# numz/ComfyUI-SeedVR2_VideoUpscaler

Measured on AMD Instinct MI355X. Metric: upscaled frames/sec (720p->4K, SeedVR2-3B), higher is better.
Workload: dtype bf16; 1 GPU; cfg3: SeedVR2-3B 32-frame 720p->4K clip (padded to 33 = 4n+1 for encode + DiT, 32 decoded), VAE tiled 1024/128; vae_tiled=True, parallelism=dp1, weights=random-init SeedVR2-3B + video_vae_v3 architecture (seeded)

## Files before the change

### comfyui-seedvr2_videoupscaler_amd/csrc/svr_api.hip

```cpp
#include "svr_common.h"
#include "../../include/seedvr2_hip.h"
#include <cstdio>
#include <vector>
#include <algorithm>
#include <cstring>

#include "svr_gemm.hip"
#include "svr_conv_halo2.hip"
#include "svr_conv_sub.hip"
#include "svr_conv_thinout.hip"
#include "svr_attn_win.hip"
#include "svr_attn.hip"
#include "svr_elementwise.hip"
#include "svr_calibrate.hip"

using namespace svr;

static thread_local char g_err[512] = "";

static int fail(const char* msg) {
    snprintf(g_err, sizeof(g_err), "%s", msg);
    return -1;
}
static int check(int hip_status, const char* what) {
    if (hip_status == 0) return 0;
    snprintf(g_err, sizeof(g_err), "%s: %s", what, hipGetErrorString((hipError_t)hip_status));
    return hip_status;
}
static inline unsigned blocks_for(int64_t n, int per) { return (unsigned)((n + per - 1) / per); }

extern "C" {

const char* svr_last_error(void) { return g_err; }
int svr_abi_version(void) { return SVR_ABI_VERSION; }
#ifndef SVR_BUILD_ID
#define SVR_BUILD_ID "unknown"
#endif
static const char g_build_id[] = "SVR_BUILD_ID=" SVR_BUILD_ID;
const char* svr_build_id(void) { return g_build_id + 13; }


int64_t svr_mfma_calibrate_workspace_bytes(void) { return (int64_t)device_cu_count() * 4 * 512 * (int64_t)sizeof(float); }

int svr_mfma_calibrate(void* workspace, int32_t iters, double* flops, void* stream) {
    StreamDeviceGuard on_stream_device(stream);
    if (!workspace || iters <= 0) return fail("svr_mfma_calibrate: workspace of svr_mfma_calibrate_workspace_bytes() and iters > 0");
    const unsigned grid = (unsigned)device_cu_count() * 4;
    hipLaunchKernelGGL(mfma_calibrate_kernel, dim3(grid), dim3(512), 0, (hipStream_t)stream, (float*)workspace, iters);
    if (flops) *flops = (double)grid * 8.0 * 16.0 * (2.0 * 32 * 32 * 16) * (double)iters;
    return check(hipGetLastError(), "svr_mfma_calibrate");
}

int svr_set_option(const char* key, int32_t value) {
    if (!key) return fail("svr_set_option: null key");
    if (!strcmp(key, "pipe_abl")) { g_pipe_abl = value; return 0; }
    if (!strcmp(key, "conv_impl")) { g_conv_impl = value; return 0; }
    if (!strcmp(key, "gemm_epi")) { g_gemm_epi = value; return 0; }
    if (!strcmp(key, "gemm_w4")) { g_gemm_w4 = value; return 0; }
    if (!strcmp(key, "gemm_w4r")) { if ((unsigned)value > 1u) return fail("svr_set_option: gemm_w4r is 0 or 1"); g_gemm_w4r = value; return 0; }
    if (!strcmp(key, "conv_rows")) { g_conv_rows = value; return 0; }
    if (!strcmp(key, "conv_band")) { g_conv_band = value; return 0; }
    if (!strcmp(key, "conv_sub")) { g_conv_sub = value; return 0; }
    if (!strcmp(key, "conv_lds")) { g_conv_lds_dbg = value; return 0; }
    if (!strcmp(key, "conv_thinout4")) { g_conv_thinout4 = value; return 0; }
    if (!strcmp(key, "attn_impl")) { g_attn_impl = value; return 0; }
    if (!strcmp(key, "attn_variant")) { g_attn_variant = value; return 0; }
    return fail("svr_set_option: unknown key");
}

int svr_device_info(char* buf, int32_t buflen) {
    int dev = 0;
    if (hipGetDevice(&dev) != hipSuccess) return fail("svr_device_info: no HIP device");
    hipDeviceProp_t p;
    if (hipGetDeviceProperties(&p, dev) != hipSuccess) return fail("svr_device_info: hipGetDeviceProperties failed");
    if (buf && buflen > 0)
        snprintf(buf, buflen, "%s arch=%s CUs=%d LDS/block=%zu mem=%.1fGB", p.name, p.gcnArchName,
                 p.multiProcessorCount, (size_t)p.maxSharedMemoryPerMultiProcessor, p.totalGlobalMem / 1e9);
    return strstr(p.gcnArchName, "gfx950") ? 0 : fail("svr_device_info: current device is not gfx950");
}

int svr_gemm_bf16(const svr_gemm_args* args, void* stream) {
    StreamDeviceGuard on_stream_device(stream);
    if (!args) return fail("svr_gemm_bf16: null args");
    const char* why = nullptr;
    const int rc = gemm_dispatch(*args, (hipStream_t)stream, &why);
    if (why) return fail(why);
    return check(rc, "svr_gemm_bf16");
}

int32_t svr_gemm_kernel_class(const svr_gemm_args* args) {
    if (!args) { fail("svr_gemm_kernel_class: null args"); return -1; }
    const char* why = nullptr;
    const int cls = gemm_route(*args, &why);
    if (why) fail(why);
    return cls;
}

const char* svr_gemm_kernel_name(int32_t cls) {
    switch (cls) {
        case SVR_KERNEL_NONE: return "none";
        case SVR_KERNEL_GEMM: return "svr::gemm_kernel";
        case SVR_KERNEL_GEMM_PERSISTENT: return "svr::gemm_w4r_kernel";
        case SVR_KERNEL_CONV_HALO: return "svr::conv_halo2_kernel";
        case SVR_KERNEL_CONV_SUBPIXEL: return "svr::conv_sub_kernel";
        case SVR_KERNEL_CONV_THIN_IN: return "svr::conv_halo2_kernel<8, 2> (thin input)";
        case SVR_KERNEL_CONV_THIN_OUT: return "svr::conv_thinout_kernel";
        case SVR_KERNEL_CONV_GENERIC: return "svr::gemm_kernel<..., CONV>";
        default: return "invalid";
    }
}

int32_t svr_gemm_gn_blocks(const svr_gemm_args* args) {
    if (!args || !args->conv.enabled || args->gn_groups <= 0) return 0;
    return conv_gn_blocks(*args);
}

int svr_groupnorm_reduce(const void* partial, double* stats, int32_t T, int32_t nblk, int32_t groups, void* stream) {
    StreamDeviceGuard on_stream_device(stream);
    if (T <= 0 || nblk <= 0) return 0;
    if (groups <= 0 || groups > 65535) return fail("svr_groupnorm_reduce: 1..65535 groups");
    if (!partial || !stats) return fail("svr_groupnorm_reduce: null pointer");
    hipLaunchKernelGGL(groupnorm_reduce_kernel, dim3(T, groups), dim3(256), 0, (hipStream_t)stream,
                       (const double2*)partial, stats, (int)nblk, groups);
    return check(hipGetLastError(), "svr_groupnorm_reduce");
}

int svr_rmsnorm_mod(const void* x, void* y, int64_t rows, int32_t dim, float eps, const float* w, const float* scale,
                    const float* shift, int32_t x_f32, void* stream) {
    StreamDeviceGuard on_stream_device(stream);
    if (rows <= 0) return 0;
    if (dim <= 0 || dim % 8 || dim > 64 * 8 * 8) return fail("svr_rmsnorm_mod: dim must be a multiple of 8 and <= 4096");
    if (!x || !y) return fail("svr_rmsnorm_mod: null pointer");
    if ((unsigned)x_f32 > (unsigned)SVR_STORE_H16) return fail("svr_rmsnorm_mod: x_f32 must be SVR_STORE_BF16 / _FP32 / _H16");
    const unsigned grid = (unsigned)(rows < 4 * 2048 ? blocks_for(rows, 4) : 2048);
    const int nc = (dim + 511) / 512;
#define SVR_RMS_LAUNCH(NC) do { if (x_f32 == SVR_STORE_FP32) hipLaunchKernelGGL((rmsnorm_mod_kernel<NC, 1>), dim3(grid), dim3(256), 0, (hipStream_t)stream, \
                                              x, (bf16_t*)y, rows, dim, eps, w, scale, shift); \
                           else if (x_f32 == SVR_STORE_H16) hipLaunchKernelGGL((rmsnorm_mod_kernel<NC, 2>), dim3(grid), dim3(256), 0, (hipStream_t)stream, \
                                              x, (bf16_t*)y, rows, dim, eps, w, scale, shift); \
                           else hipLaunchKernelGGL((rmsnorm_mod_kernel<NC, 0>), dim3(grid), dim3(256), 0, (hipStream_t)stream, \
                                              x, (bf16_t*)y, rows, dim, eps, w, scale, shift); } while (0)
    switch (nc) {
        case 1: SVR_RMS_LAUNCH(1); break; case 2: SVR_RMS_LAUNCH(2); break; case 3: SVR_RMS_LAUNCH(3); break;
        case 4: SVR_RMS_LAUNCH(4); break; case 5: SVR_RMS_LAUNCH(5); break; case 6: SVR_RMS_LAUNCH(6); break;
        case 7: SVR_RMS_LAUNCH(7); break; default: SVR_RMS_LAUNCH(8); break;
    }
#undef SVR_RMS_LAUNCH
    return check(hipGetLastError(), "svr_rmsnorm_mod");
}

int svr_ada_combine(const void* emb, const void* params, const int32_t* slot, float* out, int32_t n_vec, int32_t dim,
                    void* stream) {
    StreamDeviceGuard on_stream_device(stream);
    if (n_vec <= 0 || dim <= 0) return 0;
    if (n_vec > 65535) return fail("svr_ada_combine: at most 65535 vectors per call");
    if (!emb || !params || !slot || !out) return fail("svr_ada_combine: null pointer");
    hipLaunchKernelGGL(ada_combine_kernel, dim3(blocks_for(dim, 256), n_vec), dim3(256), 0, (hipStream_t)stream,
                       (const bf16_t*)emb, (const bf16_t*)params, slot, out, n_vec, dim);
    return check(hipGetLastError(), "svr_ada_combine");
}

int svr_qknorm_rope(void* qkv, int64_t rows, int32_t heads, const int16_t* pos, int32_t t_offset, const float* cos_tab,
                    const float* sin_tab, int32_t n_pos, int32_t n_freq, const float* wq, const float* wk, float eps,
                    void* stream) {
// ... 200 lines not shown
```

### comfyui-seedvr2_videoupscaler_amd/csrc/svr_attn.hip

```cpp
#include "svr_common.h"
#include "../../include/seedvr2_hip.h"
#include <cstdlib>

namespace svr {

template <int D, int QSUB, int KT>
__global__ __launch_bounds__(256) void attn_kernel(
    const bf16_t* __restrict__ qkv, int64_t ld_qkv, bf16_t* __restrict__ out, int64_t ld_out,
    const int32_t* __restrict__ seq_rows, const int32_t* __restrict__ out_rows,
    const int32_t* __restrict__ cu, int heads, float scale_log2) {
    constexpr int QB = 64 * QSUB;
    constexpr int DS = D / 32;
    constexpr int DB = D / 16;
    constexpr int KB = KT / 16;
    constexpr int KG = KT / 32;
    constexpr int KCH = D / 8;
    constexpr int VCH = KT / 8;
    constexpr int VSH = (VCH == 8) ? 1 : 2;
    constexpr int K_BYTES = KT * D * 2;

    extern __shared__ __attribute__((aligned(16))) char smem[];
    char* sK = smem;
    char* sV = smem + K_BYTES;

// ... 49 lines not shown
#pragma unroll
            for (int it = 0; it < MT / 256; ++it) {
                const int mt = it * 256 + tid;
                const int dc = mt % (D / 8);
                const int kq = mt / (D / 8);
                uint4 v[4];
#pragma unroll
                for (int i = 0; i < 4; ++i) {
                    const int row = seq_rows[beg + min(kt0 + 4 * kq + i, L - 1)];
                    v[i] = *(const uint4*)(vbase + (int64_t)row * ld_qkv + dc * 8);
                }
                const int G = kq >> 3, kb = (kq >> 2) & 1, gq = kq & 3;
                const int cc = G * 4 + gq;
                const uint32_t* w0 = (const uint32_t*)&v[0];
                const uint32_t* w1 = (const uint32_t*)&v[1];
                const uint32_t* w2 = (const uint32_t*)&v[2];
                const uint32_t* w3 = (const uint32_t*)&v[3];
#pragma unroll
                for (int e = 0; e < 8; ++e) {
                    const int d = dc * 8 + e;
                    const int sh = (e & 1) * 16;
                    uint2 t;
                    t.x = ((w0[e >> 1] >> sh) & 0xffffu) | (((w1[e >> 1] >> sh) & 0xffffu) << 16);
                    t.y = ((w2[e >> 1] >> sh) & 0xffffu) | (((w3[e >> 1] >> sh) & 0xffffu) << 16);
                    const int ccs = cc ^ ((d >> VSH) & (VCH - 1));
                    *(uint2*)(sV + d * (KT * 2) + ccs * 16 + kb * 8) = t;
                }
            }
        }
        __syncthreads();

        f32x4 sacc[QSUB][KB];
#pragma unroll
        for (int s = 0; s < QSUB; ++s)
#pragma unroll
            for (int kb = 0; kb < KB; ++kb) sacc[s][kb] = f32x4{0.f, 0.f, 0.f, 0.f};
#pragma unroll
        for (int ds = 0; ds < DS; ++ds) {
#pragma unroll
            for (int kb = 0; kb < KB; ++kb) {
                const int key = kb * 16 + ql;
                const int c = 4 * ds + g;
                const int slot = (c & ~15) | ((c ^ key) & 15);
                const bf16x8 kf = *(const bf16x8*)(sK + key * (D * 2) + slot * 16);
#pragma unroll
                for (int s = 0; s < QSUB; ++s)
                    sacc[s][kb] = __builtin_amdgcn_mfma_f32_16x16x32_bf16(kf, qf[s][ds], sacc[s][kb], 0, 0, 0);
            }
        }

        bf16x8 pf[QSUB][KG];
#pragma unroll
        for (int s = 0; s < QSUB; ++s) {
            float mx = -INFINITY;
#pragma unroll
            for (int kb = 0; kb < KB; ++kb)
#pragma unroll
                for (int r = 0; r < 4; ++r) {
                    const int key = kt0 + kb * 16 + 4 * g + r;
                    float v = sacc[s][kb][r] * scale_log2;
                    v = key < L ? v : -INFINITY;
                    sacc[s][kb][r] = v;
                    mx = fmaxf(mx, v);
                }
            mx = fmaxf(mx, __shfl_xor(mx, 16, 64));
            mx = fmaxf(mx, __shfl_xor(mx, 32, 64));
            const float m_new = fmaxf(m_run[s], mx);
            const float alpha = fast_exp2(m_run[s] - m_new);
            m_run[s] = m_new;
            float psum = 0.f;
#pragma unroll
            for (int kg = 0; kg < KG; ++kg) {
                float p[8];
#pragma unroll
                for (int r = 0; r < 4; ++r) {
                    p[r] = fast_exp2(sacc[s][2 * kg][r] - m_new);
                    p[4 + r] = fast_exp2(sacc[s][2 * kg + 1][r] - m_new);
                }
#pragma unroll
                for (int r = 0; r < 8; ++r) psum += p[r];
                const uint4 pk = pack8(p);
                pf[s][kg] = __builtin_bit_cast(bf16x8, pk);
            }
            l_run[s] = l_run[s] * alpha + psum;
#pragma unroll
            for (int db = 0; db < DB; ++db) {
                o[s][db][0] *= alpha; o[s][db][1] *= alpha; o[s][db][2] *= alpha; o[s][db][3] *= alpha;
            }
        }

#pragma unroll
        for (int db = 0; db < DB; ++db) {
#pragma unroll
            for (int kg = 0; kg < KG; ++kg) {
                const int d = db * 16 + ql;
                const int cc = (kg * 4 + g) ^ ((d >> VSH) & (VCH - 1));
                const bf16x8 vf = *(const bf16x8*)(sV + d * (KT * 2) + cc * 16);
#pragma unroll
                for (int s = 0; s < QSUB; ++s)
                    o[s][db] = __builtin_amdgcn_mfma_f32_16x16x32_bf16(vf, pf[s][kg], o[s][db], 0, 0, 0);
            }
        }
    }

#pragma unroll
    for (int s = 0; s < QSUB; ++s) {
        float l = l_run[s];
        l += __shfl_xor(l, 16, 64);
        l += __shfl_xor(l, 32, 64);
        if (qpos[s] >= L) continue;
        const float inv = 1.0f / l;
        const int row = out_rows[beg + qpos[s]];
        bf16_t* op = out + (int64_t)row * ld_out + (int64_t)head * D + 4 * g;
#pragma unroll
        for (int db = 0; db < DB; ++db) {
            uint2 t;
            t.x = pack2bf(o[s][db][0] * inv, o[s][db][1] * inv);
            t.y = pack2bf(o[s][db][2] * inv, o[s][db][3] * inv);
            *(uint2*)(op + 16 * db) = t;
        }
    }
}

template <int D, int QSUB, int KT>
static int launch_attn(const void* qkv, int64_t ld_qkv, void* out, int64_t ld_out, const int32_t* seq_rows,
                       const int32_t* out_rows, const int32_t* cu, int n_seq, int max_len, int heads,
                       float scale, hipStream_t s) {
    constexpr int QB = 64 * QSUB;
    const size_t lds = (size_t)KT * D * 2 * 2;
    auto kern = attn_kernel<D, QSUB, KT>;
    static uint64_t lds_attr_done = 0;
    {
        const int e = (lds > 48 * 1024) ? set_max_dynamic_lds((const void*)kern, (int)lds, lds_attr_done) : 0;
        if (e != 0) return e;
    }
    dim3 grid((max_len + QB - 1) / QB, heads, n_seq);
    hipLaunchKernelGGL(kern, grid, dim3(256), lds, s, (const bf16_t*)qkv, ld_qkv, (bf16_t*)out, ld_out,
                       seq_rows, out_rows, cu, heads, scale * 1.4426950408889634f);
    return (int)hipGetLastError();
}

int g_attn_impl = 0;

int attn_dispatch(const void* qkv, int64_t ld_qkv, void* out, int64_t ld_out, const int32_t* seq_rows,
                  const int32_t* out_rows, const int32_t* cu, int n_seq, int max_len, int heads, int head_dim,
                  float scale, hipStream_t s, const char** why) {
    *why = nullptr;
    if (n_seq <= 0 || max_len <= 0) return 0;
    if (n_seq > 65535 || heads > 65535) { *why = "svr_attn_varlen: grid too large"; return -1; }
    if (head_dim == 128 && max_len <= AW_MAXL && (ld_qkv % 8) == 0 && g_attn_impl != 1)
        return launch_attn_win(qkv, ld_qkv, out, ld_out, seq_rows, out_rows, cu, n_seq, max_len, heads, scale, s);
    if (head_dim == 128)
        return launch_attn<128, 2, 64>(qkv, ld_qkv, out, ld_out, seq_rows, out_rows, cu, n_seq, max_len, heads, scale, s);
    if (head_dim == 512)
        return launch_attn<512, 1, 32>(qkv, ld_qkv, out, ld_out, seq_rows, out_rows, cu, n_seq, max_len, heads, scale, s);
    *why = "svr_attn_varlen: head_dim must be 128 or 512";
    return -1;
}

}
```

### comfyui-seedvr2_videoupscaler_amd/vae.py

```python
import math
import os
from dataclasses import dataclass, field
from typing import Dict, List, Optional, Tuple

import torch

from .config import VAEConfig
from . import subpixel
from .ops import EPI_BIAS, EPI_RESID_GATE, Conv3dGeom, PhaseScatter, PixelShuffleGeom
from .packing import BF16, pack_conv3d, pack_matrix, pack_vec

BF16 = torch.bfloat16


@dataclass
class _Conv:
    name: str
    w: torch.Tensor
    b: torch.Tensor
    cin: int
    cout: int
    k: Tuple[int, int, int]
    stride: Tuple[int, int, int] = (1, 1, 1)
    pad_lo: int = 1
    pad_hi: int = 1
    thin: bool = False
    w_frag: Optional[torch.Tensor] = None
    head: Optional["_Conv"] = None


@dataclass
class _Norm:
    gamma: torch.Tensor
    beta: torch.Tensor


@dataclass
class _Resnet:
    norm1: _Norm
    conv1: _Conv
    norm2: _Norm
    conv2: _Conv
    shortcut: Optional[_Conv]


@dataclass
class _Attn:
    norm: _Norm
    qkv_w: torch.Tensor
    qkv_b: torch.Tensor
    out_w: torch.Tensor
    out_b: torch.Tensor
    dim: int


@dataclass
class _Up:
    upscale_w: torch.Tensor
    upscale_b: torch.Tensor
    conv: _Conv
    temporal: bool
    C: int
    merged: Optional[dict] = None


def _tile_ranges(total: int, tile: int, overlap: int) -> List[Tuple[int, int]]:
    stride = max(1, tile - overlap)
    out = []
    for s in range(0, total, stride):
        e = min(s + tile, total)
        if s > 0 and (e - s) <= overlap:
            continue
        out.append((s, e))
    return out


def _edge_weights(length: int, ov: int, fade_lo: bool, fade_hi: bool, ramp: Optional[torch.Tensor]) -> torch.Tensor:
    w = torch.ones(length, dtype=torch.float32)
    ov = max(0, min(ov, length - 1))
    if ov > 0:
        if fade_lo:
            w[:ov] = ramp[:ov]
        if fade_hi:
            w[-ov:] = 1 - ramp[:ov]
    return w


def _cos_ramp(n: int) -> Optional[torch.Tensor]:
    if n <= 0:
        return None
    return 0.5 - 0.5 * torch.cos(torch.linspace(0, 1, steps=n, dtype=torch.float32) * math.pi)


class VideoVAEEngine:
    def __init__(self, cfg: VAEConfig, state_dict: Dict[str, torch.Tensor], ops,
                 act_budget_bytes: Optional[int] = None, merge_upsamplers: bool = True, merge_causal_head: bool = True,
                 trunk_fp32: Optional[bool] = None, branch_fp32: Optional[bool] = None, tile_streams: int = 1,
                 trunk_store: Optional[str] = None, branch_store: Optional[str] = None, overflow_guard: bool = True):
        self.cfg, self.ops = cfg, ops
        kinds = {"bf16": None, "h16": torch.float16, "fp32": torch.float32}
        default = "h16" if getattr(ops, "act_dtype", BF16) == BF16 else "bf16"
        if trunk_store is None:
            trunk_store = default if trunk_fp32 is None else ("fp32" if trunk_fp32 else "bf16")
        if branch_store is None:
            branch_store = (default if trunk_store != "bf16" else "bf16") if branch_fp32 is None else \
                ("fp32" if (branch_fp32 and trunk_store != "bf16") else "bf16")
        self.trunk_store, self.branch_store = trunk_store, branch_store
        self.trunk_dtype, self.branch_dtype = kinds[trunk_store], kinds[branch_store]
        self.overflow_guard = bool(overflow_guard)
        self.overflow_reruns = 0
        self.device = ops.device
        self.tile_streams = int(tile_streams)
        self.act_budget_bytes = self._resolve_act_budget(act_budget_bytes, ops.device, self.tile_streams)
        self.sample_dtype = None
        self._streams = []
        self._edges = {}
        sd, dev = state_dict, ops.device
        ch = cfg.block_out_channels
        n = len(ch)

        def conv(name, stride=(1, 1, 1), pad=(1, 1), cin_pad=None, w=None):
            w = sd[name + ".weight"] if w is None else w
            co, ci, kt, kh, kw = w.shape
            thin = ci < 64
            if thin:
                cin_pad = cin_pad or (ci + 3) // 4 * 4
            wp = pack_conv3d(w, dev, cin_pad)
            frag = None
            if (kh, kw) == (3, 3) and tuple(stride) == (1, 1, 1) and tuple(pad) == (1, 1) and not thin \
                    and hasattr(ops, "pack_conv_frag"):
                frag = ops.pack_conv_frag(wp, kt, ci, co)
            head = None
            if merge_causal_head and kt == 3 and tuple(stride) == (1, 1, 1) and not thin:
                wsum = w.to(device=dev, dtype=BF16).float().sum(2)
                hi = wsum.to(BF16).float()
                head = conv(name, stride, pad, w=torch.stack([hi, wsum - hi], 2))
            return _Conv(name, wp, pack_vec(sd[name + ".bias"], dev),
                         cin_pad or ci, co, (kt, kh, kw), stride, pad[0] if kh > 1 else 0, pad[1] if kh > 1 else 0, thin, frag,
                         head)

        def norm(name):
            return _Norm(pack_vec(sd[name + ".weight"], dev), pack_vec(sd[name + ".bias"], dev))

        def resnet(name):
            sc = conv(name + ".conv_shortcut", pad=(0, 0)) if (name + ".conv_shortcut.weight") in sd else None
            rb = _Resnet(norm(name + ".norm1"), conv(name + ".conv1"), norm(name + ".norm2"), conv(name + ".conv2"), sc)
            if sc is None and rb.conv1.cin != rb.conv2.cout:
                raise KeyError(f"{name}: width changes {rb.conv1.cin} -> {rb.conv2.cout} but {name}.conv_shortcut is missing "
                               "from the state dict (ResnetBlock3D, attn_video_vae.py:292-305)")
            return rb

        def attn(name):
            c = sd[name + ".to_q.weight"].shape[0]
            wqkv = torch.cat([sd[name + f".{k}.weight"] for k in ("to_q", "to_k", "to_v")], dim=0)
            bqkv = torch.cat([sd[name + f".{k}.bias"] for k in ("to_q", "to_k", "to_v")], dim=0)
            return _Attn(norm(name + ".group_norm"), pack_matrix(wqkv, dev), pack_vec(bqkv, dev),
                         pack_matrix(sd[name + ".to_out.0.weight"], dev), pack_vec(sd[name + ".to_out.0.bias"], dev), c)

        def mid(name):
            return (resnet(name + ".resnets.0"), attn(name + ".attentions.0"), resnet(name + ".resnets.1"))

        self.attn_as_gemm = True
        self.enc_conv_in = conv("encoder.conv_in", cin_pad=4)
        self.enc_down = []
        for i in range(n):
            res = [resnet(f"encoder.down_blocks.{i}.resnets.{j}") for j in range(cfg.layers_per_block)]
            down = None
            if i != n - 1:
                temporal = i >= n - cfg.temporal_scale_num - 1
                down = conv(f"encoder.down_blocks.{i}.downsamplers.0.conv",
                            stride=(2 if temporal else 1, 2, 2), pad=(0, 1))
            self.enc_down.append((res, down))
        self.enc_mid = mid("encoder.mid_block")
        self.enc_norm_out = norm("encoder.conv_norm_out")
        self.enc_conv_out = conv("encoder.conv_out")
        self.dec_conv_in = conv("decoder.conv_in")
        self.dec_mid = mid("decoder.mid_block")
        self.dec_up = []
        for i in range(n):
            res = [resnet(f"decoder.up_blocks.{i}.resnets.{j}") for j in range(cfg.layers_per_block + 1)]
            up = None
            if i != n - 1:
                u = f"decoder.up_blocks.{i}.upsamplers.0"
                w = sd[u + ".upscale_conv.weight"]
                up = _Up(pack_matrix(w.reshape(w.shape[0], w.shape[1]), dev), pack_vec(sd[u + ".upscale_conv.bias"], dev),
                         conv(u + ".conv"), i < cfg.temporal_scale_num, w.shape[1])
                if merge_upsamplers and w.shape[1] % 64 == 0:
                    rz = 2 if up.temporal else 1
                    w1 = w.reshape(w.shape[0], w.shape[1]).to(device=dev, dtype=BF16)
                    b1 = sd[u + ".upscale_conv.bias"].to(device=dev, dtype=BF16)
                    w3, b3 = sd[u + ".conv.weight"].to(device=dev, dtype=BF16), sd[u + ".conv.bias"].to(device=dev, dtype=BF16)
                    up.merged = {}
                    for i in (range(5) if up.temporal else (w3.shape[2] - 1,)):
                        sig = subpixel.signature(i, rz, w3.shape[2])
                        if sig not in up.merged:
                            srcs, parts = subpixel.merge_upsampler(w1, b1, w3, b3, rz, sig)
                            packed = []
                            for py, px, wm, b, bb in parts:
                                wp = pack_conv3d(wm, dev)
                                frag = ops.pack_conv_frag(wp, len(srcs), w.shape[1], w3.shape[0], taps=(2, 2)) \
                                    if hasattr(ops, "pack_conv_frag") else None
                                packed.append((py, px, wp, b.contiguous(), bb.contiguous(), frag))
                            up.merged[sig] = (len(srcs), packed)
            self.dec_up.append((res, up))
        self.dec_norm_out = norm("decoder.conv_norm_out")
        self.dec_conv_out = conv("decoder.conv_out")
        self._iota = {}

    def parameters(self):
        seen = set()

        def walk(o):
            if torch.is_tensor(o):
                if o.is_floating_point() and id(o) not in seen:
                    seen.add(id(o))
                    yield o
            elif isinstance(o, dict):
                for v in o.values():
                    yield from walk(v)
            elif isinstance(o, (list, tuple)):
                for v in o:
                    yield from walk(v)
            elif hasattr(o, "__dataclass_fields__"):
                for f in o.__dataclass_fields__:
                    yield from walk(getattr(o, f))
        for name, v in vars(self).items():
            if name not in ("ops", "cfg") and not name.startswith("_"):
                yield from walk(v)

    def eval(self):
        return self

    def requires_grad_(self, flag: bool = False):
        return self

    def to(self, *args, **kwargs):
        dev = next((a for a in args if isinstance(a, (str, torch.device))), kwargs.get("device"))
        if dev is not None and torch.device(dev).type != self.device.type:
            raise NotImplementedError(f"{type(self).__name__} weights are resident on {self.device} (pre-tiled for the MFMA kernels); "
                                      "build a new engine on the target device instead of moving this one")
        return self

    @property
    def dtype(self):
        return self.ops.act_dtype

    def _conv(self, cw: _Conv, x: torch.Tensor, st: dict, first: bool, resid: Optional[torch.Tensor] = None,
              gn: bool = False, wide: bool = False):
        ops = self.ops
        odt = wide if isinstance(wide, torch.dtype) else (self.trunk_dtype if wide else None)
        T, H, W, Cin = x.shape
        assert Cin == cw.cin, (cw.name, Cin, cw.cin)
        if first and cw.head is not None:
            return self._conv_causal_head(cw, x, st, resid, gn, odt)
        kt, kh, kw = cw.k
        sT, sH, sW = cw.stride
        carry = kt - sT
        halo = None if first else st.get(cw.name)
        pt = (kt - 1) if first else (halo.shape[0] if halo is not None else 0)
        if not first and carry > 0 and halo is None:
            raise RuntimeError(f"{cw.name}: missing temporal halo for a non-initial slice")
        assert (T + pt - kt) % sT == 0, (cw.name, T, pt)
        To = (T + pt - kt) // sT + 1
        Ho = (H + cw.pad_lo + cw.pad_hi - kh) // sH + 1
        Wo = (W + cw.pad_lo + cw.pad_hi - kw) // sW + 1
        geom = Conv3dGeom(T, H, W, Cin, To, Ho, Wo, cw.k, cw.stride, (pt, cw.pad_lo, cw.pad_lo), halo)
        if resid is not None and tuple(resid.shape) != (To, Ho, Wo, cw.cout):
            raise ValueError(f"{cw.name}: residual {tuple(resid.shape)} does not match the output {(To, Ho, Wo, cw.cout)}")
        out = ops.empty(To, Ho, Wo, cw.cout, dtype=odt)
        f32 = out.dtype in (torch.float32, torch.float16)
        K = cw.w.shape[1]
        epi = EPI_RESID_GATE if resid is not None else EPI_BIAS
        stats = None
        fused_thin = (cw.thin and cw.cin == 4 and tuple(cw.k[1:]) == (3, 3) and tuple(cw.stride) == (1, 1, 1) and K == 128
                      and cw.cout % 128 == 0 and (cw.pad_lo, cw.pad_hi) == (1, 1))
        if cw.thin and not fused_thin:
            cols = ops.empty(To * Ho * Wo, K)
            ops.im2col_causal(x, cols, geom)
            ops.gemm(cols, cw.w, out, N=cw.cout, K=K, M=To * Ho * Wo, bias=cw.b, epilogue=epi, resid=resid,
                     lda=K, ldc=cw.cout, ldr=cw.cout, out_f32=f32)
        elif tuple(cw.k) == (1, 1, 1) and tuple(cw.stride) == (1, 1, 1) and cw.pad_lo == 0 and not gn and K == Cin:
            M_ = To * Ho * Wo
            ops.gemm(x.reshape(M_, Cin), cw.w, out.reshape(M_, cw.cout), N=cw.cout, K=K, M=M_, bias=cw.b, epilogue=epi,
                     resid=None if resid is None else resid.reshape(M_, cw.cout), out_f32=f32)
        else:
            r = ops.gemm(x, cw.w, out, N=cw.cout, K=K, bias=cw.b, epilogue=epi, resid=resid, conv=geom,
                         ldc=cw.cout, ldr=cw.cout, gn_groups=self.cfg.norm_num_groups if gn else 0,
                         W_frag=None if cw.thin else cw.w_frag, out_f32=f32)
            stats = r[1] if gn else None
        if carry > 0 and not st.get("__last_slice__", False):
            if T >= carry:
                st[cw.name] = x[T - carry:].clone()
            else:
                prev = halo if halo is not None else x[:1].expand(pt, H, W, Cin)
                st[cw.name] = torch.cat([prev, x], dim=0)[-carry:].contiguous()
        return (out, stats) if gn else out

    def _conv_causal_head(self, cw: _Conv, x, st, resid, gn, odt=None):
        T, H, W, _ = x.shape
        if resid is not None and tuple(resid.shape) != (T, H, W, cw.cout):
            raise ValueError(f"{cw.name}: residual {tuple(resid.shape)} does not match the output {(T, H, W, cw.cout)}")
        out = self.ops.empty(T, H, W, cw.cout, dtype=odt)
        stats = []
        for sub, n_in, o in ((cw.head, 1, 0), (cw, T, 1)):
            To = n_in + 1 - sub.k[0] + 1
            if To <= 0:
                continue
            geom = Conv3dGeom(n_in, H, W, cw.cin, To, H, W, sub.k, (1, 1, 1), (1, cw.pad_lo, cw.pad_lo), None)
            r = resid[o:o + To] if resid is not None else None
            res = self.ops.gemm(x[:n_in], sub.w, out[o:o + To], N=cw.cout, K=sub.w.shape[1], bias=cw.b,
                                epilogue=EPI_RESID_GATE if r is not None else EPI_BIAS, resid=r, conv=geom,
                                ldc=cw.cout, ldr=cw.cout, gn_groups=self.cfg.norm_num_groups if gn else 0, W_frag=sub.w_frag,
                                out_f32=out.dtype in (torch.float32, torch.float16))
            if gn:
                stats.append(res[1])
        if not st.get("__last_slice__", False):
            carry = cw.k[0] - 1
            st[cw.name] = x[T - carry:].clone() if T >= carry else torch.cat([x[:1].expand(carry - T, H, W, cw.cin), x], 0).contiguous()
        if not gn:
            return out
        return out, (None if any(s is None for s in stats) else torch.cat(stats, 0))

    def _gn(self, nm: _Norm, x: torch.Tensor, silu: bool, stats: Optional[torch.Tensor] = None):
        ops, cfg = self.ops, self.cfg
        if stats is None:
            stats = ops.empty(x.shape[0], cfg.norm_num_groups, 2, dtype=torch.float64)
            ops.groupnorm_stats(x, stats, cfg.norm_num_groups)
        out = ops.empty(*x.shape)
        ops.groupnorm_apply(x, out, stats, nm.gamma, nm.beta, cfg.norm_num_groups, cfg.norm_eps, silu)
        return out

    def _resnet(self, rb: _Resnet, x, st, first, x_stats=None, wide=True):
        h = self._gn(rb.norm1, x, True, x_stats)
        h, hs = self._conv(rb.conv1, h, st, first, gn=True, wide=self.branch_dtype if self.branch_dtype is not None else False)
        h = self._gn(rb.norm2, h, True, hs)
        if rb.shortcut is not None and x.dtype != self.ops.act_dtype:
            raise RuntimeError(f"{rb.shortcut.name}: a shortcut conv reads its block input as an MFMA operand; the producer must store it "
                               f"in the activation dtype, got {x.dtype}")
        sc = self._conv(rb.shortcut, x, st, first, wide=True) if rb.shortcut is not None else x
        return self._conv(rb.conv2, h, st, first, resid=sc, gn=True, wide=wide)

    def _attention(self, ab: _Attn, x):
        ops = self.ops
        T, H, W, Cc = x.shape
        n = H * W
        y = self._gn(ab.norm, x, False)
        out = ops.empty(T, H, W, Cc, dtype=self.trunk_dtype)
        if self.attn_as_gemm and n <= 65536 and n % 64 == 0:
            rb = min(n, 16384)
            npad = (n + 255) // 256 * 256
            q, v = ops.empty(T * n, Cc), ops.empty(T * n, Cc)
            k = ops.empty(T * n + npad, Cc)
            y2 = y.reshape(T * n, Cc)
            for dst, j in ((q, 0), (k, 1), (v, 2)):
                ops.gemm(y2, ab.qkv_w[j * Cc:(j + 1) * Cc], dst[:T * n], N=Cc, K=Cc, bias=ab.qkv_b[j * Cc:(j + 1) * Cc].contiguous())
            S = ops.empty(rb, n, dtype=torch.float32)
            P = ops.empty(rb, n)
            att = ops.empty(T * n, Cc)
            for t in range(T):
                vt = v[t * n:(t + 1) * n].t().contiguous()
                for r0 in range(0, n, rb):
                    r1 = min(r0 + rb, n)
                    ops.gemm(q[t * n + r0:t * n + r1], k[t * n:t * n + npad], S[:r1 - r0], N=n, K=Cc, out_f32=True)
                    ops.softmax_rows(S[:r1 - r0], P[:r1 - r0], 1.0 / math.sqrt(Cc))
                    ops.gemm(P[:r1 - r0], vt, att[t * n + r0:t * n + r1], N=Cc, K=n)
        else:
            qkv = ops.empty(T * n, 3 * Cc)
            ops.gemm(y.reshape(T * n, Cc), ab.qkv_w, qkv, N=3 * Cc, K=Cc, bias=ab.qkv_b)
            key = (T, n)
            if key not in self._iota:
                self._iota[key] = (torch.arange(T * n, dtype=torch.int32, device=self.device),
                                   (torch.arange(T + 1, dtype=torch.int32, device=self.device) * n).contiguous())
            rows, cu = self._iota[key]
            att = ops.empty(T * n, Cc)
            ops.attn_varlen(qkv, att, rows, rows, cu, n, 1, Cc, 1.0 / math.sqrt(Cc))
        ops.gemm(att, ab.out_w, out, N=Cc, K=Cc, M=T * n, bias=ab.out_b, epilogue=EPI_RESID_GATE,
                 resid=x, ldc=Cc, ldr=Cc, out_f32=out.dtype in (torch.float32, torch.float16))
        return out

    def _mid(self, m, x, st, first, x_stats=None, wide=True):
        x, _ = self._resnet(m[0], x, st, first, x_stats)
        x = self._attention(m[1], x)
        return self._resnet(m[2], x, st, first, wide=wide)

    def _upsample(self, up: _Up, x, st, first, wide=False):
        ops = self.ops
        T, H, W, Cc = x.shape
        if up.merged is not None:
            return self._upsample_subpixel(up, x, st, first, wide)
        rz = 2 if up.temporal else 1
        drop = up.temporal and first
        To = T * rz - (1 if drop else 0)
        y = ops.empty(To, 2 * H, 2 * W, Cc)
        ops.gemm(x.reshape(T * H * W, Cc), up.upscale_w, y, N=4 * rz * Cc, K=Cc, M=T * H * W, bias=up.upscale_b,
                 ps=PixelShuffleGeom(T, H, W, rz, Cc, drop))
        return self._conv(up.conv, y, st, first, gn=True, wide=wide)

    def _upsample_subpixel(self, up: _Up, x, st, first, wide=False):
        ops, cw = self.ops, up.conv
        T, H, W, Cc = x.shape
        rz = 2 if up.temporal else 1
        kt = cw.k[0]
        key = cw.name + "#subpixel"
        t0 = 0 if first else st.get(key + "#frames")
        mem = None if first else st.get(key)
        if not first and (t0 is None or mem is None):
            raise RuntimeError(f"{cw.name}: missing temporal state for a non-initial slice")
        carry = kt - 1 if rz == 1 else 1
        outs = [subpixel.output_frames(t0 + tl, rz) for tl in range(T)]
        y = ops.empty(sum(len(o) for o in outs), 2 * H, 2 * W, cw.cout, dtype=self.trunk_dtype if wide else None)
        f32 = y.dtype in (torch.float32, torch.float16)
        shared = {"frames": y.shape[0]} if hasattr(ops, "gn_shared_stats") else None

        def launch(sig, a, b, base, t_stride):
            n_src, parts = up.merged[sig]
            pt = n_src - 1
            if pt == 0:
                halo = None
            elif a >= pt:
                halo = x[a - pt:a]
            elif mem is None:
                halo = None if a == 0 else torch.cat([x[:1].expand(pt - a, H, W, Cc), x[:a]], 0).contiguous()
            else:
                halo = mem[mem.shape[0] - pt:] if a == 0 else torch.cat([mem[mem.shape[0] - (pt - a):], x[:a]], 0).contiguous()
            geom_in = x[a:b]
            if len(parts) == 4 and all(pp[5] is not None for pp in parts) and getattr(ops, "phase_quad", False):
                py, px, w, bias, bb, frag = parts[0]
                geom = Conv3dGeom(b - a, H, W, Cc, b - a, H, W, (n_src, 2, 2), (1, 1, 1), (pt, 1 - py, 1 - px), halo)
                kw = {}
                if shared is not None:
                    shared["frame0"] = base
                    kw = dict(gn_groups=self.cfg.norm_num_groups, gn_shared=shared)
                ops.gemm(geom_in, w, y[base:], N=cw.cout, K=w.shape[1], bias=bias, conv=geom,
                         phase=PhaseScatter(py, px, bb, t_stride, quad=list(parts)), W_frag=frag, out_f32=f32, **kw)
                return
            for py, px, w, bias, bb, frag in parts:
                geom = Conv3dGeom(b - a, H, W, Cc, b - a, H, W, (n_src, 2, 2), (1, 1, 1), (pt, 1 - py, 1 - px), halo)
                kw = {}
                if shared is not None:
                    shared["frame0"] = base
                    kw = dict(gn_groups=self.cfg.norm_num_groups, gn_shared=shared)
                ops.gemm(geom_in, w, y[base:], N=cw.cout, K=w.shape[1], bias=bias, conv=geom,
                         phase=PhaseScatter(py, px, bb, t_stride), W_frag=frag, out_f32=f32, **kw)

        if rz == 1:
            launch(subpixel.signature(kt - 1, 1, kt), 0, T, 0, 1)
        else:
            base, tl = 0, 0
            while tl < T:
                tg = t0 + tl
                if tg == 0:
                    launch(subpixel.signature(0, 2, kt), tl, tl + 1, base, 1)
                    base, tl = base + 1, tl + 1
                elif tg == 1:
                    launch(subpixel.signature(1, 2, kt), tl, tl + 1, base, 1)
                    launch(subpixel.signature(2, 2, kt), tl, tl + 1, base + 1, 1)
                    base, tl = base + 2, tl + 1
                else:
                    launch(subpixel.signature(3, 2, kt), tl, T, base, 2)
                    launch(subpixel.signature(4, 2, kt), tl, T, base + 1, 2)
                    base, tl = base + 2 * (T - tl), T
        if not st.get("__last_slice__", False):
            st[key + "#frames"] = t0 + T
            if carry > 0:
                if T >= carry:
                    st[key] = x[T - carry:].clone()
                else:
                    prev = mem if mem is not None else x[:1].expand(carry, H, W, Cc)
                    st[key] = torch.cat([prev, x], dim=0)[-carry:].contiguous()
        return y, (ops.gn_shared_stats(shared) if shared is not None else None)

    def _encoder_slice(self, x, st, first):
        levels = self.enc_down
        feeds_shortcut = lambda i: i < len(levels) and levels[i][0][0].shortcut is not None
        h, hs = self._conv(self.enc_conv_in, x, st, first, gn=True, wide=not feeds_shortcut(0))
        for i, (res, down) in enumerate(levels):
            for j, rb in enumerate(res):
                h, hs = self._resnet(rb, h, st, first, hs, wide=not (down is not None and j == len(res) - 1))
            if down is not None:
                h, hs = self._conv(down, h, st, first, gn=True, wide=not feeds_shortcut(i + 1))
        h, hs = self._mid(self.enc_mid, h, st, first, hs)
        h = self._gn(self.enc_norm_out, h, True, hs)
        return self._conv(self.enc_conv_out, h, st, first)

    def _decoder_slice(self, z, st, first):
        h, hs = self._conv(self.dec_conv_in, z, st, first, gn=True, wide=True)
        levels = self.dec_up
        h, hs = self._mid(self.dec_mid, h, st, first, hs, wide=levels[0][0][0].shortcut is None)
        for i, (res, up) in enumerate(levels):
            for j, rb in enumerate(res):
                h, hs = self._resnet(rb, h, st, first, hs, wide=not (up is not None and j == len(res) - 1))
            if up is not None:
                h, hs = self._upsample(up, h, st, first, wide=levels[i + 1][0][0].shortcut is None)
                if i == self.cfg.temporal_scale_num - 1 and st.get("__keep__") is not None:
                    done = st["__produced__"]
                    st["__produced__"] = done + h.shape[0]
                    n = max(1, min(h.shape[0], st["__keep__"] - done))
                    if n < h.shape[0]:
                        if not st.get("__last_slice__", False):
                            raise RuntimeError("keep_frames cuts a temporal slice that is not the clip's last one")
                        h, hs = h[:n], (hs[:n] if hs is not None else None)
# ... 232 lines not shown
```

Baseline: 3.536 frames/s.

## Add fused single-pass head_dim-512 flash attention kernel for VAE mid-block attention

New measurement: 3.570 frames/s, median of 6. Within noise of the previous version (+1.0%).

```diff
diff --git a/comfyui-seedvr2_videoupscaler_amd/csrc/svr_api.hip b/comfyui-seedvr2_videoupscaler_amd/csrc/svr_api.hip
--- a/comfyui-seedvr2_videoupscaler_amd/csrc/svr_api.hip
+++ b/comfyui-seedvr2_videoupscaler_amd/csrc/svr_api.hip
@@ -10,6 +10,7 @@
 #include "svr_conv_sub.hip"
 #include "svr_conv_thinout.hip"
 #include "svr_attn_win.hip"
+#include "svr_attn_d512.hip"
 #include "svr_attn.hip"
 #include "svr_elementwise.hip"
 #include "svr_calibrate.hip"
diff --git a/comfyui-seedvr2_videoupscaler_amd/csrc/svr_attn.hip b/comfyui-seedvr2_videoupscaler_amd/csrc/svr_attn.hip
--- a/comfyui-seedvr2_videoupscaler_amd/csrc/svr_attn.hip
+++ b/comfyui-seedvr2_videoupscaler_amd/csrc/svr_attn.hip
@@ -225,6 +225,8 @@
         return launch_attn_win(qkv, ld_qkv, out, ld_out, seq_rows, out_rows, cu, n_seq, max_len, heads, scale, s);
     if (head_dim == 128)
         return launch_attn<128, 2, 64>(qkv, ld_qkv, out, ld_out, seq_rows, out_rows, cu, n_seq, max_len, heads, scale, s);
+    if (head_dim == 512 && (ld_qkv % 8) == 0 && g_attn_impl != 1)
+        return launch_attn_d512(qkv, ld_qkv, out, ld_out, seq_rows, out_rows, cu, n_seq, max_len, heads, scale, s);
     if (head_dim == 512)
         return launch_attn<512, 1, 32>(qkv, ld_qkv, out, ld_out, seq_rows, out_rows, cu, n_seq, max_len, heads, scale, s);
     *why = "svr_attn_varlen: head_dim must be 128 or 512";
diff --git a/comfyui-seedvr2_videoupscaler_amd/csrc/svr_attn_d512.hip b/comfyui-seedvr2_videoupscaler_amd/csrc/svr_attn_d512.hip
--- /dev/null
+++ b/comfyui-seedvr2_videoupscaler_amd/csrc/svr_attn_d512.hip
@@ -0,0 +1,300 @@
+#include "svr_common.h"
+#include "../../include/seedvr2_hip.h"
+
+namespace svr {
+
+constexpr int A5_D = 512;
+constexpr int A5_KT = 64;
+constexpr int A5_QB = 128;
+constexpr int A5_ROW = A5_D * 2;
+constexpr int A5_TILE = A5_KT * A5_ROW;
+constexpr int A5_LDS = 2 * A5_TILE;
+constexpr float A5_DEFER = 6.0f;
+
+template <int OFF>
+SVR_DEVICE void a5_k4(bf16x8 (&k)[4], unsigned a0, unsigned a1, unsigned a2, unsigned a3) {
+    asm volatile(
+        "ds_read_b128 %0, %4 offset:%8\n\t"
+        "ds_read_b128 %1, %5 offset:%8\n\t"
+        "ds_read_b128 %2, %6 offset:%8\n\t"
+        "ds_read_b128 %3, %7 offset:%8"
+        : "=&v"(k[0]), "=&v"(k[1]), "=&v"(k[2]), "=&v"(k[3])
+        : "v"(a0), "v"(a1), "v"(a2), "v"(a3), "n"(OFF)
+        : "memory");
+}
+template <int OFF>
+SVR_DEVICE void a5_tr8(bf16x4 (&v)[8], unsigned a0, unsigned a1, unsigned a2, unsigned a3) {
+    asm volatile(
+        "ds_read_b64_tr_b16 %0, %8 offset:%12\n\t"
+        "ds_read_b64_tr_b16 %1, %8 offset:%13\n\t"
+        "ds_read_b64_tr_b16 %2, %9 offset:%12\n\t"
+        "ds_read_b64_tr_b16 %3, %9 offset:%13\n\t"
+        "ds_read_b64_tr_b16 %4, %10 offset:%12\n\t"
+        "ds_read_b64_tr_b16 %5, %10 offset:%13\n\t"
+        "ds_read_b64_tr_b16 %6, %11 offset:%12\n\t"
+        "ds_read_b64_tr_b16 %7, %11 offset:%13"
+        : "=&v"(v[0]), "=&v"(v[1]), "=&v"(v[2]), "=&v"(v[3]), "=&v"(v[4]), "=&v"(v[5]), "=&v"(v[6]), "=&v"(v[7])
+        : "v"(a0), "v"(a1), "v"(a2), "v"(a3), "n"(OFF), "n"(OFF + 8 * A5_ROW)
+        : "memory");
+}
+
+SVR_DEVICE void a5_barrier_landed() {
+    __builtin_amdgcn_s_waitcnt(0x0F70);
+    __builtin_amdgcn_s_barrier();
+    asm volatile("" ::: "memory");
+}
+
+SVR_DEVICE void a5_mfma_first(f32x16& acc, const bf16x8& a, const bf16x8& b) {
+    asm volatile("v_mfma_f32_32x32x16_bf16 %0, %1, %2, 0" : "=&v"(acc) : "v"(a), "v"(b));
+}
+SVR_DEVICE void a5_mfma_acc(f32x16& acc, const bf16x8& a, const bf16x8& b) {
+    asm volatile("v_mfma_f32_32x32x16_bf16 %0, %1, %2, %0" : "+v"(acc) : "v"(a), "v"(b));
+}
+SVR_DEVICE void a5_mfma_o(f32x16& acc, const bf16x8& a, const bf16x8& b) {
+    asm volatile("v_mfma_f32_32x32x16_bf16 %0, %1, %2, %0" : "+a"(acc) : "v"(a), "v"(b));
+}
+SVR_DEVICE void a5_mfma_settle_o(f32x16& o0, f32x16& o1, f32x16& o2, f32x16& o3) {
+    asm volatile("s_nop 15\n\ts_nop 7" : "+a"(o0), "+a"(o1), "+a"(o2), "+a"(o3));
+}
+SVR_DEVICE void a5_scale_o(f32x16& acc, float alpha) {
+    f32x16 t = acc;
+    asm volatile("" : "+v"(t));
+#pragma unroll
+    for (int r = 0; r < 16; ++r) t[r] *= alpha;
+    asm volatile("" : "+v"(t));
+    acc = t;
+    asm volatile("" : "+a"(acc));
+}
+SVR_DEVICE void a5_mfma_settle(f32x16& s0, f32x16& s1) {
+    asm volatile("s_nop 15\n\ts_nop 7" : "+v"(s0), "+v"(s1));
+}
+
+__global__ __launch_bounds__(256, 1) void attn_d512_kernel(
+    const bf16_t* __restrict__ qkv, int64_t ld_qkv, bf16_t* __restrict__ out, int64_t ld_out,
+    const int32_t* __restrict__ seq_rows, const int32_t* __restrict__ out_rows, const int32_t* __restrict__ cu,
+    int heads, int n_items, int items_per_xcd, int qt_per_pair, float scale_log2) {
+    extern __shared__ __attribute__((aligned(16))) char smem[];
+
+    const int bid = blockIdx.x;
+    const int item = (bid & 7) * items_per_xcd + (bid >> 3);
+    if (item >= n_items) return;
+    const int pair = item / qt_per_pair;
+    const int seq = pair / heads, head = pair - seq * heads;
+    const int beg = cu[seq];
+    const int L = cu[seq + 1] - beg;
+    const int q0 = (item - pair * qt_per_pair) * A5_QB;
+    if (q0 >= L) return;
+
+    const int tid = threadIdx.x, lane = tid & 63;
+    const int wave = __builtin_amdgcn_readfirstlane(tid >> 6);
+    const int l31 = lane & 31, hi = lane >> 5;
+    const int nk = (L + A5_KT - 1) / A5_KT;
+
+    const int64_t ld_bytes = ld_qkv * 2;
+    const char* qbase = (const char*)qkv + (int64_t)head * A5_ROW;
+    const int64_t k_off = (int64_t)heads * A5_ROW, v_off = 2 * k_off;
+
+    auto tile_rows = [&](int t) -> int {
+        const int tt = min(t, nk - 1);
+        return seq_rows[beg + min(tt * A5_KT + wave * 16 + (lane & 15), L - 1)];
+    };
+    auto stage_k = [&](int idx) __attribute__((always_inline)) {
+        unsigned ln = lane;
+        asm volatile("" : "+v"(ln));
+#pragma unroll
+        for (int i = 0; i < 16; ++i) {
+            const int64_t row = __builtin_amdgcn_readlane(idx, i);
+            glds16(qbase + row * ld_bytes + k_off + ((ln ^ i) << 4), smem + (wave * 16 + i) * A5_ROW);
+        }
+    };
+    auto stage_v = [&](int idx) __attribute__((always_inline)) {
+        unsigned ln = lane;
+        asm volatile("" : "+v"(ln));
+#pragma unroll
+        for (int i = 0; i < 16; ++i) {
+            const int64_t row = __builtin_amdgcn_readlane(idx, i);
+            glds16(qbase + row * ld_bytes + v_off + ((ln ^ ((i & 3) << 2)) << 4), smem + A5_TILE + (wave * 16 + i) * A5_ROW);
+        }
+    };
+    int idx_cur = tile_rows(0);
+    stage_k(idx_cur);
+
+    const int qpos = q0 + wave * 32 + l31;
+    bf16x8 qf[32];
+    {
+        const char* qp = qbase + (int64_t)seq_rows[beg + min(qpos, L - 1)] * ld_bytes + hi * 16;
+#pragma unroll
+        for (int ds = 0; ds < 32; ++ds) qf[ds] = *(const bf16x8*)(qp + ds * 32);
+    }
+    int idx_nxt = tile_rows(1);
+
+    const unsigned lds_base = (unsigned)(uintptr_t)(__attribute__((address_space(3))) char*)smem;
+    unsigned ka_[8];
+#pragma unroll
+    for (int ds = 0; ds < 8; ++ds) ka_[ds] = lds_base + l31 * A5_ROW + (((2 * ds + hi) ^ (l31 & 15)) << 4);
+    const int i16 = lane & 15, G = (lane >> 4) & 1, jr = i16 >> 2, c4 = i16 & 3;
+    unsigned va_[4];
+#pragma unroll
+    for (int m = 0; m < 4; ++m)
+        va_[m] = lds_base + A5_TILE + (hi * 4 + jr) * A5_ROW + (((((m ^ jr) << 2) | (2 * G + (c4 >> 1))) << 4)) + (c4 & 1) * 8;
+
+    f32x16 o[16];
+    float m_run = -INFINITY, l_run = 0.f;
+#pragma unroll
+    for (int m = 0; m < 16; ++m)
+#pragma unroll
+        for (int r = 0; r < 16; ++r) o[m][r] = 0.f;
+
+    a5_barrier_landed();
+
+    f32x16 sacc[2];
+    bf16x8 pf[2][2];
+    bf16x8 kA[4], kB[4];
+    bf16x4 vA[8], vB[8];
+
+#define A5_QK(K, G)                                                                                                    \
+        _Pragma("unroll") for (int e = 0; e < 4; ++e) {                                                               \
+            if (((G) & 7) == 0 && e == 0) a5_mfma_first(sacc[(G) >> 3], K[e], qf[4 * ((G) & 7) + e]);                \
+            else a5_mfma_acc(sacc[(G) >> 3], K[e], qf[4 * ((G) & 7) + e]);                                            \
+        }
+#define A5_KOFF(G) ((((G) >> 3) * 32 * A5_ROW) + ((((G) & 7) >> 1) * 256))
+#define A5_KREAD(K, G) a5_k4<A5_KOFF(G)>(K, ka_[4 * ((G) & 1) + 0], ka_[4 * ((G) & 1) + 1], ka_[4 * ((G) & 1) + 2], ka_[4 * ((G) & 1) + 3]);
+#define A5_QK2(G)                                       \
+        aw_wait_k<4>(kA); A5_QK(kA, G)     A5_KREAD(kA, (G) + 2)                                                      \
+        aw_wait_k<4>(kB); A5_QK(kB, (G) + 1) A5_KREAD(kB, (G) + 3)
+    auto qk_tile = [&]() __attribute__((always_inline)) {
+        A5_KREAD(kA, 0)
+        A5_KREAD(kB, 1)
+        A5_QK2(0) A5_QK2(2) A5_QK2(4) A5_QK2(6) A5_QK2(8) A5_QK2(10) A5_QK2(12)
+        aw_wait_k<4>(kA); A5_QK(kA, 14)
+        aw_wait_k<0>(kB); A5_QK(kB, 15)
+        a5_mfma_settle(sacc[0], sacc[1]);
+    };
+
+    auto softmax_tile = [&](int t) __attribute__((always_inline)) {
+        if ((t + 1) * A5_KT > L) {
+            const int kbase = t * A5_KT + 4 * hi;
+#pragma unroll
+            for (int kb = 0; kb < 2; ++kb)
+#pragma unroll
+                for (int r = 0; r < 16; ++r)
+                    if (kbase + kb * 32 + (r & 3) + 8 * (r >> 2) >= L) sacc[kb][r] = -INFINITY;
+        }
+        float mx = sacc[0][0];
+#pragma unroll
+        for (int kb = 0; kb < 2; ++kb)
+#pragma unroll
+            for (int r = 0; r < 16; ++r) mx = fmaxf(mx, sacc[kb][r]);
+        mx = aw_other_half_max(mx);
+        if (!__all((mx - m_run) * scale_log2 <= A5_DEFER)) {
+            const float m_new = fmaxf(m_run, mx);
+            const float alpha = fast_exp2((m_run - m_new) * scale_log2);
+            m_run = m_new;
+            l_run *= alpha;
+#pragma unroll
+            for (int m = 0; m < 16; ++m) a5_scale_o(o[m], alpha);
+        }
+        const float mc = m_run * scale_log2;
+        float ps = 0.f;
+#pragma unroll
+        for (int kb = 0; kb < 2; ++kb)
+#pragma unroll
+            for (int u = 0; u < 2; ++u) {
+                float p[8];
+#pragma unroll
+                for (int e = 0; e < 8; ++e) {
+                    p[e] = fast_exp2(__builtin_fmaf(sacc[kb][8 * u + e], scale_log2, -mc));
+                    ps += p[e];
+                }
+                const uint4 pk = pack8(p);
+                pf[kb][u] = __builtin_bit_cast(bf16x8, pk);
+            }
+        l_run += ps;
+    };
+
+#define A5_PV(V, G)                                                                                                    \
+        _Pragma("unroll") for (int m = 0; m < 4; ++m) {                                                              \
+            const bf16x8 vf = __builtin_shufflevector(V[2 * m], V[2 * m + 1], 0, 1, 2, 3, 4, 5, 6, 7);               \
+            a5_mfma_o(o[4 * ((G) & 3) + m], vf, pf[(G) >> 3][((G) >> 2) & 1]);                                        \
+        }
+#define A5_VOFF(G) ((((G) >> 2) * 16 * A5_ROW) + (((G) & 3) * 256))
+#define A5_VREAD(V, G) a5_tr8<A5_VOFF(G)>(V, va_[0], va_[1], va_[2], va_[3]);
+#define A5_PV2(G)                                                                                                      \
+        aw_wait_lgkm<8>(vA); A5_PV(vA, G)     A5_VREAD(vA, (G) + 2)                                                   \
+        aw_wait_lgkm<8>(vB); A5_PV(vB, (G) + 1) A5_VREAD(vB, (G) + 3)
+    auto pv_tile = [&]() __attribute__((always_inline)) {
+        A5_PV2(0) A5_PV2(2) A5_PV2(4) A5_PV2(6) A5_PV2(8) A5_PV2(10) A5_PV2(12)
+        aw_wait_lgkm<8>(vA); A5_PV(vA, 14)
+        aw_wait_lgkm<0>(vB); A5_PV(vB, 15)
+        a5_mfma_settle_o(o[12], o[13], o[14], o[15]);
+    };
+
+    for (int t = 0; t < nk; ++t) {
+        stage_v(idx_cur);
+        qk_tile();
+        a5_barrier_landed();
+        if (t + 1 < nk) stage_k(idx_nxt);
+        A5_VREAD(vA, 0)
+        softmax_tile(t);
+        A5_VREAD(vB, 1)
+        pv_tile();
+        idx_cur = idx_nxt;
+        idx_nxt = tile_rows(t + 2);
+        a5_barrier_landed();
+    }
+#undef A5_QK
+#undef A5_KOFF
+#undef A5_KREAD
+#undef A5_QK2
+#undef A5_PV
+#undef A5_VOFF
+#undef A5_VREAD
+#undef A5_PV2
+
+    {
+        const float l = aw_other_half_sum(l_run);
+        const float inv = 1.0f / l;
+        unsigned tl = threadIdx.x;
+        asm volatile("" : "+v"(tl));
+        const int qp2 = q0 + (tl >> 6) * 32 + (tl & 31);
+        const bool valid = qp2 < L;
+        const int orow = valid ? out_rows[beg + qp2] : 0;
+        char* op = (char*)out + ((int64_t)orow * ld_out + (int64_t)head * A5_D) * 2 + ((tl >> 5) & 1) * 16;
+#pragma unroll
+        for (int m = 0; m < 16; ++m) {
+            f32x16 t = o[m];
+            asm volatile("" : "+v"(t));
+#pragma unroll
+            for (int rq = 0; rq < 4; rq += 2) {
+                uint32_t ax = pack2bf(t[4 * rq + 0] * inv, t[4 * rq + 1] * inv);
+                uint32_t ay = pack2bf(t[4 * rq + 2] * inv, t[4 * rq + 3] * inv);
+                uint32_t bx = pack2bf(t[4 * rq + 4] * inv, t[4 * rq + 5] * inv);
+                uint32_t by = pack2bf(t[4 * rq + 6] * inv, t[4 * rq + 7] * inv);
+                const u32x2 sx = __builtin_amdgcn_permlane32_swap(ax, bx, false, false);
+                const u32x2 sy = __builtin_amdgcn_permlane32_swap(ay, by, false, false);
+                if (valid) *(uint4*)(op + (32 * m + 8 * rq) * 2) = make_uint4(sx[0], sy[0], sx[1], sy[1]);
+            }
+        }
+    }
+}
+
+static int launch_attn_d512(const void* qkv, int64_t ld_qkv, void* out, int64_t ld_out, const int32_t* seq_rows,
+                            const int32_t* out_rows, const int32_t* cu, int n_seq, int max_len, int heads, float scale,
+                            hipStream_t s) {
+    auto kern = attn_d512_kernel;
+    static uint64_t lds_attr_done = 0;
+    {
+        const int e = set_max_dynamic_lds((const void*)kern, A5_LDS, lds_attr_done);
+        if (e != 0) return e;
+    }
+    const int64_t qt = (max_len + A5_QB - 1) / A5_QB;
+    const int64_t items = (int64_t)n_seq * heads * qt;
+    const int64_t per_xcd = (items + 7) / 8;
+    if (8 * per_xcd > 0x7fffffff) return -2;
+    hipLaunchKernelGGL(kern, dim3((unsigned)(8 * per_xcd)), dim3(256), A5_LDS, s, (const bf16_t*)qkv, ld_qkv, (bf16_t*)out,
+                       ld_out, seq_rows, out_rows, cu, heads, (int)items, (int)per_xcd, (int)qt,
+                       scale * 1.4426950408889634f);
+    return (int)hipGetLastError();
+}
+
+}
diff --git a/comfyui-seedvr2_videoupscaler_amd/vae.py b/comfyui-seedvr2_videoupscaler_amd/vae.py
--- a/comfyui-seedvr2_videoupscaler_amd/vae.py
+++ b/comfyui-seedvr2_videoupscaler_amd/vae.py
@@ -96,7 +96,8 @@
     def __init__(self, cfg: VAEConfig, state_dict: Dict[str, torch.Tensor], ops,
                  act_budget_bytes: Optional[int] = None, merge_upsamplers: bool = True, merge_causal_head: bool = True,
                  trunk_fp32: Optional[bool] = None, branch_fp32: Optional[bool] = None, tile_streams: int = 1,
-                 trunk_store: Optional[str] = None, branch_store: Optional[str] = None, overflow_guard: bool = True):
+                 trunk_store: Optional[str] = None, branch_store: Optional[str] = None, overflow_guard: bool = True,
+                 attn_single_pass: Optional[bool] = None):
         self.cfg, self.ops = cfg, ops
         kinds = {"bf16": None, "h16": torch.float16, "fp32": torch.float32}
         default = "h16" if getattr(ops, "act_dtype", BF16) == BF16 else "bf16"
@@ -161,6 +162,12 @@
             return (resnet(name + ".resnets.0"), attn(name + ".attentions.0"), resnet(name + ".resnets.1"))
 
         self.attn_as_gemm = True
+        if attn_single_pass is None:
+            env = os.environ.get("SVR_VAE_ATTN_SINGLE_PASS", "1")
+            if env not in ("0", "1"):
+                raise ValueError(f"SVR_VAE_ATTN_SINGLE_PASS must be 0 or 1, got {env!r}")
+            attn_single_pass = env == "1"
+        self.attn_single_pass = bool(attn_single_pass)
         self.enc_conv_in = conv("encoder.conv_in", cin_pad=4)
         self.enc_down = []
         for i in range(n):
@@ -346,7 +353,8 @@
         n = H * W
         y = self._gn(ab.norm, x, False)
         out = ops.empty(T, H, W, Cc, dtype=self.trunk_dtype)
-        if self.attn_as_gemm and n <= 65536 and n % 64 == 0:
+        single_pass = self.attn_single_pass and Cc == 512 and n >= 1024
+        if self.attn_as_gemm and n <= 65536 and n % 64 == 0 and not single_pass:
             rb = min(n, 16384)
             npad = (n + 255) // 256 * 256
             q, v = ops.empty(T * n, Cc), ops.empty(T * n, Cc)
```
